# AwesomePeiweiPan/Droid-SLAM_Reserch

Hardware: AMD Instinct MI355X
Metric: BA update iters/sec (2000-edge equivalents; 256 keyframes, 48x64) (higher is better)
Workload: dtype f32; 1 GPU; 256-keyframe / 2000-edge global BA, 48x64, t0=1, lm=1e-5 ep=1e-2 (BASELINE configs[2]); edges_total=2000, solve=fp64 dense Cholesky on device, chol_failed=False

## Files before the change

droid-slam_reserch_amd/csrc/ba_internal.hpp:

```cpp
#pragma once
#include <hip/hip_runtime.h>
#include <stddef.h>
#include <stdint.h>

namespace droid {

constexpr int LIN_THREADS = 256;
constexpr int LIN_PPT = 2;
constexpr int LIN_CP = LIN_THREADS * LIN_PPT;
constexpr int LIN_WAVES = LIN_THREADS / 64;
constexpr int CHOL_NB = 64;
__host__ __device__ inline int chol_ld(int n) { return (n + 1 + 15) & ~15; }
__host__ __device__ inline size_t chol_flag_words(int n) { return 2 * ((size_t)(n + 1 + CHOL_NB - 1) / CHOL_NB) + 8; }
__host__ __device__ inline int chol_tile_index(int nrb, int bi, int bj) { return bj * nrb - bj * (bj - 1) / 2 + (bi - bj); }
__host__ __device__ inline size_t chol_tiles(int n) {
  const int nb = (n + CHOL_NB - 1) / CHOL_NB, nrb = (n + 1 + CHOL_NB - 1) / CHOL_NB;
  return (size_t)chol_tile_index(nrb, nb, nb);
}
__host__ __device__ inline size_t chol_mbuf_offset(int n) { return ((size_t)(n + CHOL_NB - 1) / CHOL_NB) * CHOL_NB * CHOL_NB; }
__host__ __device__ inline size_t chol_lfin_offset(int n) { return 2 * chol_mbuf_offset(n); }
__host__ __device__ inline size_t chol_ldiag_doubles(int n) { return chol_lfin_offset(n) + chol_tiles(n) * CHOL_NB * CHOL_NB; }

__host__ __device__ inline size_t pk_colbase(int n, int J) {
  return (size_t)CHOL_NB * ((size_t)J * (size_t)(n + 1) - (size_t)CHOL_NB * (size_t)J * (size_t)(J - 1) / 2);
}
__host__ __device__ inline int pk_width(int n, int J) { return (n - CHOL_NB * J) < CHOL_NB ? (n - CHOL_NB * J) : CHOL_NB; }
__host__ __device__ inline size_t pk_total(int n) {
  if (n <= 0) return 0;
  const int nb = (n + CHOL_NB - 1) / CHOL_NB;
  return pk_colbase(n, nb - 1) + (size_t)(n + 1 - CHOL_NB * (nb - 1)) * (size_t)pk_width(n, nb - 1);
}
__host__ __device__ inline size_t pk_index(int n, int gi, int gj) {
  const int J = gj / CHOL_NB;
  return pk_colbase(n, J) + (size_t)(gi - CHOL_NB * J) * (size_t)pk_width(n, J) + (size_t)(gj - CHOL_NB * J);
}
__host__ __device__ inline unsigned pk_index32(int n, int gi, int gj) {
  const int J = gj >> 6, c0 = J << 6;
  const int w = (n - c0) < CHOL_NB ? (n - c0) : CHOL_NB;
  return (unsigned)(CHOL_NB * (J * (n + 1) - (CHOL_NB / 2) * J * (J - 1)) + (gi - c0) * w + (gj - c0));
}

enum { HDR_STATUS = 0, HDR_M = 1, HDR_CHOL_FAIL = 2, HDR_NENT = 3, HDR_NWORK = 4,
       HDR_NC1 = 5, HDR_NC2 = 6,
       HDR_WORDS = 16 };
enum { STATUS_BAD_INDEX = 1, STATUS_ETA_ROWS = 2, STATUS_CHOL_FAIL = 4, STATUS_CHOL_STALL = 8 };

struct BaView {
  int E, nbuf, H, W, HW;
  int t0, t1, P, M;
  int n, ld;
  int nch;
  int own0, own1;
  int motion_only;
  int* hdr;
  int* slot_of;
  int* kx;
  int* seg_ptr;
  int* seg_edge;
  int* cursor;
  int* ent_ptr;
  int* ent_row;
  int* ent_pose;
  int* wk_ptr;
  int* order;
  int* xtmp;
  int* cls_list;
  int* gt_ptr;
  double* Gpart;
  int s2_split;
  float* Hpart;
  float* Q;
  float* w;
  float* Erows;
  float* Ebuf;
  float* sy_part[2];
  int sy_ns[2];
  int wide;
  int zsplit;
  float* zpart;
  double* sys;
  double* psys;
  int packed;
  double* xsol;
  float* dx;
  int* bs_flags;
  double* ldiag;
  int* hint;
  int hint_tag;
  int* ov_ready;
  float* pose_snap;
};

constexpr int SY_WGS = 1024;
constexpr int S2_WGS = 1536;
constexpr int SF_WGS = 1536;
constexpr int LIN_WGS = 1536;
constexpr int LIN_ZERO_WGS = 192;
constexpr int SF_TP = 64;
constexpr int SW_MID = 256;
constexpr int SW_BIG = 512;
constexpr int tri_tiles16(int rows) { return (rows / 16) * (rows / 16 + 1) / 2; }
constexpr int SY_T1 = tri_tiles16(SW_MID), SY_T2 = tri_tiles16(SW_BIG);
constexpr int SY_FOLD_GROUPS = SY_T1 / 4;

inline size_t ba_carve(BaView& v, void* ws, int E, int nbuf, int H, int W, int t0, int t1, int M) {
  v.E = E; v.nbuf = nbuf; v.H = H; v.W = W; v.HW = H * W;
  v.t0 = t0; v.t1 = t1; v.P = t1 - t0; v.M = M;
  v.n = 6 * v.P; v.ld = chol_ld(v.n);
  v.nch = (v.HW + LIN_CP - 1) / LIN_CP;
  v.own0 = 0; v.own1 = nbuf; v.motion_only = 0;
  v.hint = nullptr; v.hint_tag = 0;
  size_t off = 0;
  char* base = static_cast<char*>(ws);
  auto take = [&](size_t bytes) {
    void* p = base ? base + off : nullptr;
    off += (bytes + 255) & ~size_t(255);
    return p;
  };
  v.hdr = static_cast<int*>(take(sizeof(int) * HDR_WORDS));
  v.slot_of = static_cast<int*>(take(sizeof(int) * (nbuf + 1)));
  v.kx = static_cast<int*>(take(sizeof(int) * (nbuf + 1)));
  v.seg_ptr = static_cast<int*>(take(sizeof(int) * (nbuf + 2)));
  v.seg_edge = static_cast<int*>(take(sizeof(int) * (E + 1)));
  v.cursor = static_cast<int*>(take(sizeof(int) * (nbuf + 2)));
  v.ent_ptr = static_cast<int*>(take(sizeof(int) * (nbuf + 2)));
  v.ent_row = static_cast<int*>(take(sizeof(int) * ((size_t)M + E + 1)));
  v.ent_pose = static_cast<int*>(take(sizeof(int) * ((size_t)M + E + 1)));
  v.wk_ptr = static_cast<int*>(take(sizeof(int) * (nbuf + 2)));
  v.order = static_cast<int*>(take(sizeof(int) * (nbuf + 2)));
  v.gt_ptr = static_cast<int*>(take(sizeof(int) * (nbuf + 2)));
  v.cls_list = static_cast<int*>(take(sizeof(int) * 2 * (nbuf + 2)));
  v.xtmp = static_cast<int*>(take(sizeof(int) * 3 * ((size_t)E + 1)));
  v.Hpart = static_cast<float*>(take(sizeof(float) * ((size_t)E * v.nch * LIN_WAVES * 32 + 32)));
  v.Q = static_cast<float*>(take(sizeof(float) * ((size_t)M * v.HW + 4)));
  v.w = static_cast<float*>(take(sizeof(float) * ((size_t)M * v.HW + 4)));
  v.Erows = nullptr;
  v.wide = (M > 0 && (long)E >= 12l * M && (v.HW % 32) == 0) ? 1 : 0;
  v.Ebuf = nullptr;
  if (v.wide) v.Ebuf = static_cast<float*>(take(sizeof(float) * (6 * ((size_t)M + E) * v.HW + 64)));
  v.sy_part[0] = v.sy_part[1] = nullptr;
  v.sy_ns[0] = v.sy_ns[1] = 0;
  if (v.wide) {
    const int stages = v.HW / 32;
    int nsw = (SY_WGS + M - 1) / M, nsb = (256 + 4 * M - 1) / (4 * M);
    nsw = nsw < 2 ? 2 : (nsw > stages ? stages : nsw);
    nsb = nsb < 2 ? 2 : (nsb > stages ? stages : nsb);
    if (nsw > 16) nsw = 16;
    if (nsb > 16) nsb = 16;
    v.sy_ns[0] = nsw; v.sy_ns[1] = nsb;
    v.sy_part[0] = static_cast<float*>(take(sizeof(float) * ((size_t)M * nsw * SY_T1 * 256 + 64)));
    v.sy_part[1] = static_cast<float*>(take(sizeof(float) * ((size_t)M * nsb * SY_T2 * 256 + 64)));
  }
  v.zsplit = 1;
  if (M > 0) {
    const int z = LIN_WGS / (M * v.nch);
    v.zsplit = z < 1 ? 1 : (z > 8 ? 8 : z);
  }
  v.zpart = nullptr;
  if (v.zsplit > 1) v.zpart = static_cast<float*>(take(sizeof(float) * ((size_t)v.zsplit * M * 8 * v.HW + 64)));
  v.s2_split = 1;
  v.Gpart = nullptr;
  if (M > 0) {
    const int ptiles = (v.HW + 63) / 64;
    int ns = S2_WGS / M;
    v.s2_split = ns < 1 ? 1 : (ns > ptiles ? ptiles : ns);
    size_t tiles = (size_t)E * 7 / 4 + (size_t)M + 1;
    if (tiles > (size_t)28 * M) tiles = (size_t)28 * M;
    v.Gpart = static_cast<double*>(take(sizeof(double) * (tiles * v.s2_split * 256 + 64)));
  }
  v.sys = static_cast<double*>(take(sizeof(double) * ((size_t)(v.n + 1) * v.ld + 8)));
  v.psys = static_cast<double*>(take(sizeof(double) * (pk_total(v.n) + 8)));
  v.packed = 0;
  v.xsol = static_cast<double*>(take(sizeof(double) * ((size_t)v.ld + 1)));
  v.bs_flags = static_cast<int*>(take(sizeof(int) * chol_flag_words(v.n)));
  v.ldiag = static_cast<double*>(take(sizeof(double) * chol_ldiag_doubles(v.n)));
  v.dx = static_cast<float*>(take(sizeof(float) * ((size_t)v.n + 8)));
  v.ov_ready = static_cast<int*>(take(sizeof(int) * ((size_t)(v.n + 1 + CHOL_NB - 1) / CHOL_NB + 8)));
  v.pose_snap = static_cast<float*>(take(sizeof(float) * 7 * (size_t)nbuf));
  return off;
}

__host__ __device__ inline int solver_preset_words(const BaView& v) {
  return (int)((reinterpret_cast<const char*>(v.bs_flags) - reinterpret_cast<const char*>(v.xsol)) / 4 +
               (long)chol_flag_words(v.n));
}
__host__ __device__ inline int solver_preset_tiles(const BaView& v) { return v.n > 0 ? (int)chol_tiles(v.n) : 0; }

struct BaLaunchPlan {
  int zero_wgs;
  int asm_units;
  dim3 schur2;
  int sf_split;
  dim3 syrk[2], fold;
};
inline BaLaunchPlan ba_launch_plan(const BaView& v) {
  BaLaunchPlan p;
  p.zero_wgs = LIN_ZERO_WGS;
  p.asm_units = v.E > 0 ? v.E + (solver_preset_words(v) + 1023) / 1024 + solver_preset_tiles(v) : 0;
  p.schur2 = dim3(v.M + (p.asm_units + 4 * v.s2_split - 1) / (4 * v.s2_split), v.s2_split);
  const int tiles = (v.HW + SF_TP - 1) / SF_TP, ns = SF_WGS / (v.M > 0 ? v.M : 1);
  p.sf_split = ns < 1 ? 1 : (ns > tiles ? tiles : ns);
  p.syrk[0] = dim3(v.M, v.sy_ns[0], 1);
  p.syrk[1] = dim3(v.M, v.sy_ns[1], 4);
  p.fold = dim3(v.M, SY_FOLD_GROUPS, 2);
  return p;
}

struct CholSystem {
  double* S; int n, ld; double* x; int* flags; double* ldiag; int* fail;
  explicit CholSystem(const BaView& v)
      : S(v.sys), n(v.n), ld(v.ld), x(v.xsol), flags(v.bs_flags), ldiag(v.ldiag), fail(v.hdr + HDR_CHOL_FAIL) {}
  CholSystem(double* scratch, int n, double* x, int* fail);
  static size_t scratch_doubles(int n);
};

void launch_wave_reduce32_test(const float* in, float* out, hipStream_t s);
void launch_lin_test(const BaView& v, const float* poses, const float* disps, const float* intr, const float* sens,
                     const float* targets, const float* weights, const float* eta, const int64_t* ii, const int64_t* jj,
                     bool motion_only, bool ragged, hipStream_t s);
void launch_prep(const BaView& v, const int64_t* ii, const int64_t* jj, hipStream_t s);
void launch_unpack_system(const BaView& v, hipStream_t s);
void launch_build_stage(const BaView& v, const BaLaunchPlan& plan, const float* poses, const float* disps,
                        const float* intr, const float* sens, const float* targets, const float* weights,
                        const float* eta, const int64_t* ii, const int64_t* jj, bool motion_only,
                        int stage, hipStream_t s);
void launch_update(const BaView& v, float* poses, float* disps, const float* intr, const float* weights,
                   const int64_t* ii, const int64_t* jj, const double* x, float* dx_out, float* dz_out,
                   bool motion_only, hipStream_t s, int* status_mirror = nullptr);
void launch_chol_preset(const CholSystem& c, hipStream_t s);
bool launch_chol_factor(const CholSystem& c, double lm, double ep, hipStream_t s);
void launch_chol_backsolve(const CholSystem& c, bool factor_single, hipStream_t s);
void launch_chol_solve(const CholSystem& c, double lm, double ep, hipStream_t s, bool preset_done);

void launch_unpack_cols(const BaView& v, int J0, int J1, double lm, double ep, int epoch, hipStream_t s);
bool launch_chol_factor_overlap(const CholSystem& c, const int* ready, int epoch, hipStream_t s);
bool chol_overlap_available(int n);

}
```

droid-slam_reserch_amd/csrc/chol.hip:

```cpp
#include <hip/hip_runtime.h>
#include <mutex>

#include <cstdint>
#include <cstdlib>

#include "ba_internal.hpp"
#include "launchers.hpp"

namespace droid {

constexpr int NB = CHOL_NB;

#ifdef CHOL_STAMPS
__device__ unsigned long long g_chol_stamps[64 * 16];
__device__ unsigned long long g_bs_stamps[64 * 8];
__shared__ unsigned long long g_chol_lstamps[16];
extern "C" int droid_debug_chol_stamps(unsigned long long* out) {
  return (int)hipMemcpyFromSymbol(out, HIP_SYMBOL(g_chol_stamps), sizeof(unsigned long long) * 64 * 16);
}
extern "C" int droid_debug_bs_stamps(unsigned long long* out) {
  return (int)hipMemcpyFromSymbol(out, HIP_SYMBOL(g_bs_stamps), sizeof(unsigned long long) * 64 * 8);
}
#define STEP_STAMP(slot)                                                                                      \
  do { if (threadIdx.x == 0 && panel && (blockIdx.x < 2))                                                      \
// ... 821 lines not shown
  int *done = flags, *dver = flags + nrb, *abortf = flags + 2 * nrb;
  const int G = (int)gridDim.x, wg = (int)blockIdx.x, t = (int)threadIdx.x;
  const int total = (int)chol_tiles(n);
  {
    int cs = 0;
    for (int j = 0; j < nb; j++) {
      if (j >= 1 && (cs % G) == wg) cfp_publish_diag(dver, j, 0);
      cs += nrb - j;
    }
  }
  OV_STAMP_ENTERED();
  if (t == 0) {
    int nt = 0, cj = 0, cs = 0;
    for (int idx = wg; idx < total && nt < MAXT; idx += G) {
      while (idx >= cs + (nrb - cj)) {
        cs += nrb - cj;
        cj++;
      }
      s_ti[nt] = cj + (idx - cs);
      s_tj[nt] = cj;
      s_nx[nt] = cfp_first_step(cj);
      nt++;
    }
    s_nt = nt;
  }
  __syncthreads();
  while (true) {
    if (t < 64) {
      int pick = -1, spins = 0, klast = -2;
      bool ok = true;
      const int nt = s_nt;
      while (true) {
        bool any_left = false;
        for (int i = 0; i < nt; i++) {
          const int bi = s_ti[i], bj = s_tj[i], k = s_nx[i];
          if (k > bj - 1) continue;
          any_left = true;
          const bool panel = (bj == k + 1);
          const CfpInput in = cfp_input<true>(t, bi, bj, k, panel, done, dver, ready, epoch, Ldiag, n);
          const int fv = (in.flag == nullptr) ? 0x7fffffff : cfp_load(in.flag);
          const bool sat = (in.slot != nullptr) ? __double_as_longlong(gload<true>(in.slot)) != CFP_TAG : fv >= in.need;
          if (__all(sat)) {
            pick = i;
            klast = k;
            if (cfp_waits_for_done(bj, k, panel)) {
              const int d0 = __shfl(fv, 0), d1 = (bj != bi) ? __shfl(fv, 1) : d0;
              const int cok = (min(d0, d1) - 3) >> 2;
              klast = max(k, min(cok, bj - 3));
            }
            break;
          }
        }
        if (!any_left) pick = -2;
        if (pick != -1) break;
        if (++spins > (CFP_SPIN_LIMIT << 2) || ((spins & 63) == 0 && __any(cfp_load(abortf) == 1))) {
          ok = false;
          break;
        }
        __builtin_amdgcn_s_sleep(4);
      }
      if (t == 0) {
        s_pick = ok ? pick : -3;
        s_klast = klast;
        if (!ok) cfp_report_stall(fail, abortf);
      }
    }
    __syncthreads();
    const int pick = s_pick;
    if (pick < 0) return;
    const int bi = __builtin_amdgcn_readfirstlane(s_ti[pick]), bj = __builtin_amdgcn_readfirstlane(s_tj[pick]);
    const int k = __builtin_amdgcn_readfirstlane(s_nx[pick]);
    const int klast = __builtin_amdgcn_readfirstlane(s_klast);
    chol_tile_persist<true>(S, n, ld, k, bi, bj, fail, lm, ep, Ldiag, done, abortf, k == cfp_first_step(bj), klast);
    OV_STAMP_DIAG(bi, bj, k);
    if (bj != k + 1 && bi == bj) cfp_publish_diag(dver, bj, max(k, klast) + 1);
    __syncthreads();
    if (t == 0) s_nx[pick] = max(k, klast) + 1;
    __syncthreads();
  }
}

__global__ __launch_bounds__(256) void chol_backsolve_kernel(double* __restrict__ S, int n, int ld,
                                                             int k, double* __restrict__ x) {
  __shared__ double L[NB * LDP];
  __shared__ double xk[NB];
  const int t = threadIdx.x;
  const int c0 = k * NB;
  const int wk = min(NB, n - c0);
  load_tile64(DROID_LDS(L), (const gbl_f64*)S, ld, c0, c0, c0, c0 + wk, c0 + wk, true, 1.0);
  __syncthreads();
  if (t < 64) {
    double z = (t < wk) ? S[(size_t)n * ld + c0 + t] : 0.0;
    const double rinv = 1.0 / L[t * LDP + t];
#pragma unroll
    for (int i = NB - 1; i >= 0; i--) {
      const double xi = readlane_f64(z * rinv, i);
      z = (t == i) ? xi : ((t < i) ? fma(-L[i * LDP + t], xi, z) : z);
    }
    xk[t] = z;
  }
  __syncthreads();
  if (blockIdx.x == 0) {
    if (t < wk) x[c0 + t] = xk[t];
    return;
  }
  const int c = (blockIdx.x - 1) * 256 + t;
  if (c < c0) {
    double s4[4] = {0.0, 0.0, 0.0, 0.0};
    const double* col = S + (size_t)c0 * ld + c;
#pragma unroll
    for (int r = 0; r < NB; r += 16) {
      double v[16];
#pragma unroll
      for (int u = 0; u < 16; u++) v[u] = (r + u < wk) ? col[(size_t)(r + u) * ld] : 0.0;
#pragma unroll
      for (int u = 0; u < 16; u++) s4[u & 3] = fma(v[u], xk[r + u], s4[u & 3]);
    }
    S[(size_t)n * ld + c] -= (s4[0] + s4[1]) + (s4[2] + s4[3]);
  }
}

constexpr int BSP_MAX_BLOCKS = 200;
constexpr long long BSP_SENTINEL = -1LL;

__device__ __forceinline__ void load_tile64_w123(lds_f64* __restrict__ dst, const gbl_f64* __restrict__ S,
                                                 int ld, int r0, int c0, int row_end, int col_end) {
  const int t = threadIdx.x - 64;
  f64x2 v[11];
#pragma unroll
  for (int it = 0; it < 11; it++) {
    const int idx2 = it * 192 + t;
    const int i = idx2 >> 5, j = (idx2 & 31) * 2;
    const bool ok = (idx2 < 2048) && (r0 + i < row_end) && (c0 + j < col_end);
    const gbl_f64* p = S + (size_t)(ok ? r0 + i : 0) * ld + (ok ? c0 + j : 0);
    v[it] = *(const gbl_f64x2*)p;
    if (!ok) v[it] = (f64x2){0.0, 0.0};
    else if (c0 + j + 1 >= col_end) v[it][1] = 0.0;
  }
#pragma unroll
  for (int it = 0; it < 11; it++) {
    const int idx2 = it * 192 + t;
    if (idx2 < 2048) {
      const int i = idx2 >> 5, j = (idx2 & 31) * 2;
      *(lds_f64x2*)(&dst[i * LDP + j]) = v[it];
    }
  }
}

template <bool FAST>
__global__ __launch_bounds__(256) void chol_backsolve_persistent_kernel(
    double* __restrict__ S, int n, int ld, double* __restrict__ x, int* __restrict__ err,
    const double* __restrict__ Ldiag) {
  __shared__ double Ld[NB * LDP];
  __shared__ double Tt[2][NB * LDP];
  __shared__ double xk[NB];
  __shared__ int dead;
  const int t = threadIdx.x;
  const int nb = gridDim.x;
  const int j = blockIdx.x;
  const int c0 = j * NB;
  const int wj = min(NB, n - c0);
  BS_STAMP(0);
  if (t == 0) dead = 0;
  if (FAST) load_tile64(DROID_LDS(Ld), (const gbl_f64*)Ldiag + (size_t)j * NB * NB, NB, 0, 0, 0, wj, wj, true, 1.0);
  else load_tile64(DROID_LDS(Ld), (const gbl_f64*)S, ld, c0, c0, c0, c0 + wj, c0 + wj, true, 1.0);
  double z = (t < wj) ? S[(size_t)n * ld + c0 + t] : 0.0;
  int cur = 0;
  auto load_k = [&](double* dst, int k) {
    if (FAST && k == j + 1)
      load_tile64_w123(DROID_LDS(dst), (const gbl_f64*)Ldiag + chol_mbuf_offset(n) + (size_t)j * NB * NB, NB, 0, 0, NB, NB);
    else
      load_tile64_w123(DROID_LDS(dst), (const gbl_f64*)S, ld, k * NB, c0, n, c0 + wj);
  };
  if (j < nb - 1 && t >= 64) load_k(Tt[0], nb - 1);
  __syncthreads();
  double Lcol[NB];
  double Wcol[16];
  if (t < 64) {
#pragma unroll
    for (int i = FAST ? 16 : 0; i < NB; i++) Lcol[i] = Ld[i * LDP + t];
    if (FAST) {
      const int pb = t >> 4, br = pb == 3 ? 1 : 0, bc = pb == 3 ? 2 : pb + 1;
      const double* Wg = Ldiag + (size_t)j * NB * NB + (size_t)(16 * br) * NB + 16 * bc + (t & 15);
#pragma unroll
      for (int c = 0; c < 16; c++) Wcol[c] = Wg[c * NB];
    }
  }
  auto poll_matvec = [&](int k, const double (&Tc)[NB]) -> double {
    const int gi = k * NB + t;
    double xv = 0.0;
    if (gi < n) {
      int spins = 0;
      while (true) {
        xv = __hip_atomic_load(&x[gi], __ATOMIC_RELAXED, __HIP_MEMORY_SCOPE_AGENT);
        if (__double_as_longlong(xv) != BSP_SENTINEL) break;
        if (++spins > (1 << 22)) {
          dead = 1;
          atomicMax(err, 2);
          xv = 0.0;
          break;
        }
        __builtin_amdgcn_s_sleep(1);
      }
    }
    if (k == j + 1) BS_STAMP(1);
    xk[t] = xv;
    double a0 = 0.0, a1 = 0.0, a2 = 0.0, a3 = 0.0;
#pragma unroll
    for (int r = 0; r < NB; r += 4) {
      const f64x2 x01 = *(const lds_f64x2*)&DROID_LDS(xk)[r], x23 = *(const lds_f64x2*)&DROID_LDS(xk)[r + 2];
      a0 = fma(Tc[r + 0], x01[0], a0);
      a1 = fma(Tc[r + 1], x01[1], a1);
      a2 = fma(Tc[r + 2], x23[0], a2);
      a3 = fma(Tc[r + 3], x23[1], a3);
    }
    return (a0 + a1) + (a2 + a3);
  };
  const int klast = FAST ? j + 2 : j + 1;
  for (int k = nb - 1; k >= klast; k--) {
    if (t >= 64) {
      if (k - 1 > j) load_k(Tt[cur ^ 1], k - 1);
    } else {
      double Tc[NB];
      {
        const double* T = Tt[cur];
#pragma unroll
        for (int r = 0; r < NB; r++) Tc[r] = T[r * LDP + t];
      }
      z -= poll_matvec(k, Tc);
    }
    cur ^= 1;
    if (!FAST && k == j + 1) {
      BS_STAMP(2);
      break;
    }
    __syncthreads();
    if (dead) return;
  }
  BS_STAMP(3);
  if (t < 64) {
    double xsol = 0.0;
    double Mc[NB];
    if (FAST && j < nb - 1) {
      const double* T = Tt[cur];
#pragma unroll
      for (int r = 0; r < NB; r++) Mc[r] = T[r * LDP + t];
    }
    const double rinv = FAST ? 0.0 : 1.0 / Ld[t * LDP + t];
    const int rr = t & 15, rowb = t >> 4;
#define DROID_BS_STEP(B, II)                                                                            \
    {                                                                                                  \
      double zr = z * rinv, xi;                                                                        \
      asm volatile("s_nop 1\n\tv_mov_b64_dpp %0, %1 row_newbcast:" #II " row_mask:0xf bank_mask:0xf"   \
                   : "=v"(xi) : "v"(zr));                                                              \
      z = fma(-Lcol[16 * B + II], xi, z);   \
      xsol = (rr == II) ? xi : xsol;                                                                   \
    }
#define DROID_BS_WTERM(ACC, C)                                                                          \
    asm volatile("v_fmac_f64_dpp %0, %1, %2 row_newbcast:" #C " row_mask:0xf bank_mask:0xf"             \
                 : "+v"(ACC) : "v"(z), "v"(Wcol[C]));
#define DROID_BS_BLOCK(B)                                                                               \
    if (rowb == B) {                                                                                   \
      if (FAST) {                                                                                      \
        double xw = 0.0, xv2 = 0.0;                                                                    \
        asm volatile("s_nop 1" : "+v"(z));                                                             \
        DROID_BS_WTERM(xw, 0) DROID_BS_WTERM(xv2, 1) DROID_BS_WTERM(xw, 2) DROID_BS_WTERM(xv2, 3)      \
        DROID_BS_WTERM(xw, 4) DROID_BS_WTERM(xv2, 5) DROID_BS_WTERM(xw, 6) DROID_BS_WTERM(xv2, 7)      \
        DROID_BS_WTERM(xw, 8) DROID_BS_WTERM(xv2, 9) DROID_BS_WTERM(xw, 10) DROID_BS_WTERM(xv2, 11)    \
        DROID_BS_WTERM(xw, 12) DROID_BS_WTERM(xv2, 13) DROID_BS_WTERM(xw, 14) DROID_BS_WTERM(xv2, 15)  \
        xsol = xw + xv2;                                                                               \
      } else {                                                                                         \
        DROID_BS_STEP(B, 15) DROID_BS_STEP(B, 14) DROID_BS_STEP(B, 13) DROID_BS_STEP(B, 12)            \
        DROID_BS_STEP(B, 11) DROID_BS_STEP(B, 10) DROID_BS_STEP(B, 9) DROID_BS_STEP(B, 8)              \
        DROID_BS_STEP(B, 7) DROID_BS_STEP(B, 6) DROID_BS_STEP(B, 5) DROID_BS_STEP(B, 4)                \
        DROID_BS_STEP(B, 3) DROID_BS_STEP(B, 2) DROID_BS_STEP(B, 1) DROID_BS_STEP(B, 0)                \
      }                                                                                                \
      xk[t] = xsol;                                                                                    \
    }                                                                                                  \
    if (B > 0 && rowb < B) {                                                                           \
      double u0 = 0.0, u1 = 0.0;                                                                       \
      _Pragma("unroll") for (int ii = 0; ii < 16; ii += 2) {                                           \
        const f64x2 xx = *(const lds_f64x2*)&DROID_LDS(xk)[16 * B + ii];                                \
        u0 = fma(Lcol[16 * B + ii], xx[0], u0);                                                        \
        u1 = fma(Lcol[16 * B + ii + 1], xx[1], u1);                                                    \
      }                                                                                                \
      z -= u0 + u1;                                                                                    \
    }
    DROID_BS_BLOCK(3)
    DROID_BS_BLOCK(2)
    DROID_BS_BLOCK(1)
    DROID_BS_BLOCK(0)
#undef DROID_BS_BLOCK
#undef DROID_BS_WTERM
#undef DROID_BS_STEP
    BS_STAMP(2);
    if (FAST && j < nb - 1) xsol -= poll_matvec(j + 1, Mc);
    if (__double_as_longlong(xsol) == BSP_SENTINEL) xsol = __longlong_as_double(0x7ff8000000000000LL);
    BS_STAMP(4);
    if (t < wj) __hip_atomic_store(&x[c0 + t], xsol, __ATOMIC_RELAXED, __HIP_MEMORY_SCOPE_AGENT);
    BS_STAMP(5);
  }
}

struct CholSwitches {
  bool multi_launch;
  bool cooperative;
  bool force_bs_refusal;
  int grid;
  int overlap_reserve;
};
static const CholSwitches& chol_switches() {
  const auto is_set = [](const char* name) { return getenv(name) != nullptr; };
  const auto number = [](const char* name, int unset) { const char* v = getenv(name); return v ? atoi(v) : unset; };
  static const CholSwitches sw = {is_set("DROID_CHOL_MULTI_LAUNCH"), number("DROID_CHOL_COOPERATIVE", 0) != 0,
                                  is_set("DROID_CHOL_FORCE_BS_REFUSAL"), number("DROID_CHOL_GRID", 0),
                                  number("DROID_OVERLAP_RESERVE_CUS", 32)};
  return sw;
}

struct PersistState {
  hipStream_t last = nullptr;
  hipEvent_t ev = nullptr;
  bool any = false;
  int resident = -1;
};
static PersistState g_persist[64];
static std::mutex g_persist_mu;

static int chol_resident_workgroups() {
  int dev = 0;
  if (hipGetDevice(&dev) != hipSuccess || dev < 0 || dev >= 64) return 0;
  std::lock_guard<std::mutex> lock(g_persist_mu);
  int& cached = g_persist[dev].resident;
  if (cached < 0) {
    int occ = 0;
    hipDeviceProp_t prop;
    const bool known = hipGetDeviceProperties(&prop, dev) == hipSuccess &&
        hipOccupancyMaxActiveBlocksPerMultiprocessor(&occ, chol_factor_persistent_kernel<false>, 512, 0) == hipSuccess;
    cached = known ? occ * prop.multiProcessorCount : 0;
  }
  return cached;
}

static int chol_single_launch(const CholSystem& c) {
  const int nb = (c.n + NB - 1) / NB;
  if (chol_switches().multi_launch || nb < 2 || (c.ld % 16) != 0 || (reinterpret_cast<uintptr_t>(c.S) % 128) != 0) return 0;
  const int resident = chol_resident_workgroups();
  return (resident >= 8 && chol_tiles(c.n) <= (size_t)10 * resident) ? resident : 0;
}

static bool launch_spinning_grid(const void* fn, int workgroups, int threads, void** args, hipStream_t s, bool refuse = false) {
  std::lock_guard<std::mutex> lock(g_persist_mu);
  int dev = 0;
  if (hipGetDevice(&dev) == hipSuccess && dev >= 0 && dev < 64) {
    PersistState& st = g_persist[dev];
    if (st.any && st.last != s) {
      if (!st.ev && hipEventCreateWithFlags(&st.ev, hipEventDisableTiming) != hipSuccess) st.ev = nullptr;
      if (st.ev && hipEventRecord(st.ev, st.last) == hipSuccess) (void)hipStreamWaitEvent(s, st.ev, 0);
      (void)hipGetLastError();
    }
    st.last = s, st.any = true;
  }
  if (!chol_switches().cooperative) {
    (void)hipLaunchKernel(fn, dim3(workgroups), dim3(threads), args, 0, s);
    return true;
  }
  if (!refuse && hipLaunchCooperativeKernel(fn, dim3(workgroups), dim3(threads), args, 0, s) == hipSuccess) return true;
  (void)hipGetLastError();
  return false;
}

__global__ __launch_bounds__(256) void chol_ldiag_to_sys_kernel(double* __restrict__ S, int n, int ld,
                                                                const double* __restrict__ Ldiag) {
  const int j = blockIdx.x, c0 = j * NB, wk = min(NB, n - c0);
  for (int idx = threadIdx.x; idx < NB * NB; idx += blockDim.x) {
    const int i = idx / NB, c = idx % NB;
    if (i < wk && c <= i) S[(size_t)(c0 + i) * ld + c0 + c] = Ldiag[(size_t)j * NB * NB + idx];
  }
}

static bool launch_factor_grid(const void* fn, CholSystem c, double lm, double ep, const int* ready, int epoch, int cap,
                               hipStream_t s) {
  void* args[] = {&c.S, &c.n, &c.ld, &c.fail, &lm, &ep, &c.flags, &c.ldiag, &ready, &epoch};
  return launch_spinning_grid(fn, chol_tiles(c.n) < (size_t)cap ? (int)chol_tiles(c.n) : cap, 512, args, s);
}

static int chol_overlap_cap(int n) {
  const CholSwitches& sw = chol_switches();
  const int nb = (n + NB - 1) / NB;
  if (n <= 0 || sw.cooperative || sw.multi_launch || nb < 2) return 0;
  const int resident = chol_resident_workgroups();
  if (resident < 8 || chol_tiles(n) > (size_t)10 * resident) return 0;
  const int cap = resident - (sw.overlap_reserve > 0 ? sw.overlap_reserve : 0);
  return (cap >= 8 && chol_tiles(n) <= (size_t)10 * cap) ? cap : 0;
}
bool chol_overlap_available(int n) { return chol_overlap_cap(n) > 0; }

bool launch_chol_factor_overlap(const CholSystem& c, const int* ready, int epoch, hipStream_t s) {
  if (!ready || (c.ld % 16) != 0 || (reinterpret_cast<uintptr_t>(c.S) % 128) != 0) return false;
  const int cap = chol_overlap_cap(c.n);
  if (cap == 0) return false;
  return launch_factor_grid((const void*)chol_factor_persistent_kernel<true>, c, 0.0, 0.0, ready, epoch, cap, s);
}

bool launch_chol_factor(const CholSystem& c, double lm, double ep, hipStream_t s) {
  if (c.n <= 0) return false;
  if (int cap = chol_single_launch(c)) {
    const int grid = chol_switches().grid;
    if (grid >= 8 && grid < cap) cap = grid;
    if (launch_factor_grid((const void*)chol_factor_persistent_kernel<false>, c, lm, ep, nullptr, 0, cap, s)) return true;
  }
  const int nb = (c.n + NB - 1) / NB;
  const int nrb = (c.n + 1 + NB - 1) / NB;
  for (int k = -1; k + 1 < nb; k++)
    hipLaunchKernelGGL(chol_step_kernel, dim3(nrb - k - 1, k < 0 ? 2 : nb - k - 1), dim3(512), 0, s, c.S, c.n,
                       c.ld, k, c.fail, lm, ep);
  return false;
}

void launch_chol_backsolve(const CholSystem& c, bool factor_single, hipStream_t s) {
  const int nb = (c.n + NB - 1) / NB;
  if (nb >= 2 && nb <= BSP_MAX_BLOCKS) {
    CholSystem a = c;
    const double* ld_arg = factor_single ? c.ldiag : nullptr;
    void* args[] = {&a.S, &a.n, &a.ld, &a.x, &a.fail, &ld_arg};
    const void* fn = factor_single ? (const void*)chol_backsolve_persistent_kernel<true>
                                   : (const void*)chol_backsolve_persistent_kernel<false>;
    if (launch_spinning_grid(fn, nb, 256, args, s, chol_switches().force_bs_refusal)) return;
  }
  if (factor_single)
    hipLaunchKernelGGL(chol_ldiag_to_sys_kernel, dim3(nb), dim3(256), 0, s, c.S, c.n, c.ld, c.ldiag);
  for (int k = nb - 1; k >= 0; k--) {
    const int c0 = k * NB;
    hipLaunchKernelGGL(chol_backsolve_kernel, dim3(1 + (c0 + 255) / 256), dim3(256), 0, s, c.S, c.n,
                       c.ld, k, c.x);
  }
}

void launch_chol_preset(const CholSystem& c, hipStream_t s) {
  (void)hipMemsetAsync(c.fail, 0, sizeof(int), s);
  const size_t xbytes = sizeof(double) * (size_t)c.n, fbytes = sizeof(int) * chol_flag_words(c.n);
  const char* xb = reinterpret_cast<const char*>(c.x);
  const char* fb = reinterpret_cast<const char*>(c.flags);
  if (fb >= xb + xbytes && fb - xb <= (ptrdiff_t)(xbytes + 4096)) {
    (void)hipMemsetAsync(c.x, 0xFF, (size_t)(fb - xb) + fbytes, s);
  } else {
    (void)hipMemsetAsync(c.x, 0xFF, xbytes, s);
    (void)hipMemsetAsync(c.flags, 0xFF, fbytes, s);
  }
  (void)hipMemsetAsync(c.ldiag + chol_lfin_offset(c.n), 0xFF, sizeof(double) * chol_tiles(c.n) * NB * NB, s);
}

void launch_chol_solve(const CholSystem& c, double lm, double ep, hipStream_t s, bool preset_done) {
  if (c.n <= 0) return;
  if (!preset_done) launch_chol_preset(c, s);
  const bool single = launch_chol_factor(c, lm, ep, s);
  launch_chol_backsolve(c, single, s);
}

size_t CholSystem::scratch_doubles(int n) {
  if (n <= 0) return 0;
  return (size_t)(n + 1) * chol_ld(n) + chol_ldiag_doubles(n) + (chol_flag_words(n) + 1) / 2 + 16;
}
CholSystem::CholSystem(double* scratch, int n_, double* x_, int* fail_)
    : S(scratch), n(n_), ld(chol_ld(n_)), x(x_), fail(fail_) {
  ldiag = S + (size_t)(n + 1) * ld;
  flags = reinterpret_cast<int*>(ldiag + chol_ldiag_doubles(n));
}

__global__ void chol_pack_kernel(const double* __restrict__ A, const double* __restrict__ b,
                                 double* __restrict__ S, int n, int ld) {
  const size_t idx = (size_t)blockIdx.x * blockDim.x + threadIdx.x;
  if (idx >= (size_t)(n + 1) * ld) return;
  const int r = (int)(idx / ld), c = (int)(idx % ld);
  double val = 0.0;
  if (r < n && c < n) val = A[(size_t)r * n + c];
  else if (r == n && c < n) val = b[c];
  S[idx] = val;
}

void launch_chol_pack(const double* A, const double* b, double* S, int n, int ld, hipStream_t s) {
  const size_t tot = (size_t)(n + 1) * ld;
  hipLaunchKernelGGL(chol_pack_kernel, dim3((unsigned)((tot + 255) / 256)), dim3(256), 0, s, A, b,
                     S, n, ld);
}

}
```

Before: 2048 iters/s.

## Add paired-column persistent backsolve kernel with 512 threads per workgroup

Adds a new backward-substitution kernel in which each 512-thread workgroup owns two adjacent 64-column blocks instead of one. This halves the number of spinning workgroups and the cross-workgroup dependency chain. The near off-diagonal tiles are preloaded and multiplied by precomputed diagonal inverses with f64 MFMA, so the coupling between the two columns is resolved locally. It is enabled by default whenever the single-launch factor path is used. In exchange it uses more registers and LDS per workgroup, and the polling and sentinel logic is more complex.

```diff
diff --git a/droid-slam_reserch_amd/csrc/ba_internal.hpp b/droid-slam_reserch_amd/csrc/ba_internal.hpp
--- a/droid-slam_reserch_amd/csrc/ba_internal.hpp
+++ b/droid-slam_reserch_amd/csrc/ba_internal.hpp
@@ -20,6 +20,9 @@
 __host__ __device__ inline size_t chol_mbuf_offset(int n) { return ((size_t)(n + CHOL_NB - 1) / CHOL_NB) * CHOL_NB * CHOL_NB; }
 __host__ __device__ inline size_t chol_lfin_offset(int n) { return 2 * chol_mbuf_offset(n); }
 __host__ __device__ inline size_t chol_ldiag_doubles(int n) { return chol_lfin_offset(n) + chol_tiles(n) * CHOL_NB * CHOL_NB; }
+__host__ __device__ inline int chol_bs_pairs_grid(int nb) { return (nb + 1) / 2; }
+__host__ __device__ inline int chol_bs_pairs_owner(int col) { return col / 2; }
+__host__ __device__ inline int chol_bs_pairs_first(int wg) { return 2 * wg; }
 
 __host__ __device__ inline size_t pk_colbase(int n, int J) {
   return (size_t)CHOL_NB * ((size_t)J * (size_t)(n + 1) - (size_t)CHOL_NB * (size_t)J * (size_t)(J - 1) / 2);
diff --git a/droid-slam_reserch_amd/csrc/chol.hip b/droid-slam_reserch_amd/csrc/chol.hip
--- a/droid-slam_reserch_amd/csrc/chol.hip
+++ b/droid-slam_reserch_amd/csrc/chol.hip
@@ -1147,19 +1147,304 @@
   }
 }
 
+#ifdef CHOL_STAMPS
+#define BS_STAMP_W(slot, wv) do { if (threadIdx.x == 64 * (wv) && blockIdx.x < 64) g_bs_stamps[blockIdx.x * 8 + (slot)] = wall_clock64(); } while (0)
+#else
+#define BS_STAMP_W(slot, wv) do { } while (0)
+#endif
+
+struct BspTileRegs { f64x2 v[4]; };
+__device__ __forceinline__ BspTileRegs bsp_tile_issue(const gbl_f64* __restrict__ src, size_t pitch, int rows_valid) {
+  const int t = threadIdx.x;
+  BspTileRegs r;
+#pragma unroll
+  for (int it = 0; it < 4; it++) {
+    const int idx2 = it * 512 + t, i = idx2 >> 5, j = (idx2 & 31) * 2;
+    const bool ok = i < rows_valid;
+    r.v[it] = *(const gbl_f64x2*)(src + (ok ? (size_t)i * pitch + j : 0));
+    if (!ok) r.v[it] = (f64x2){0.0, 0.0};
+  }
+  return r;
+}
+__device__ __forceinline__ void bsp_tile_store(lds_f64* __restrict__ dst, const BspTileRegs& r) {
+  const int t = threadIdx.x;
+#pragma unroll
+  for (int it = 0; it < 4; it++) {
+    const int idx2 = it * 512 + t, i = idx2 >> 5, j = (idx2 & 31) * 2;
+    *(lds_f64x2*)(&dst[i * LDP + j]) = r.v[it];
+  }
+}
+
+constexpr int BSP_DC = 10 * 256;
+__device__ __forceinline__ int bsp_dc_source(int e) {
+  const int blk = e >> 7, i = (e & 127) >> 3, j = (e & 7) * 2;
+  int br, bc;
+  if (blk < 6) {
+    br = blk < 1 ? 1 : (blk < 3 ? 2 : 3);
+    bc = blk - br * (br - 1) / 2;
+  } else {
+    br = blk == 9 ? 1 : 0;
+    bc = blk == 9 ? 2 : blk - 5;
+  }
+  return (16 * br + i) * NB + 16 * bc + j;
+}
+
+__device__ __forceinline__ void bsp_times_inverse(lds_f64* T, const lds_f64* D, int g, int lane) {
+  const int fr = lane & 15, fg = lane >> 4;
+#pragma unroll
+  for (int q = 3; q >= 0; q--) {
+    lds_f64* Cq = &T[(16 * g) * LDP + 16 * q];
+    f64x4 acc;
+#pragma unroll
+    for (int i = 0; i < 4; i++) acc[i] = Cq[(fg + 4 * i) * LDP + fr];
+#pragma unroll
+    for (int s2 = q + 1; s2 < 4; s2++)
+#pragma unroll
+      for (int kk = 0; kk < 16; kk += 4)
+        acc = __builtin_amdgcn_mfma_f64_16x16x4f64(-T[(16 * g + fr) * LDP + 16 * s2 + kk + fg],
+                                                   D[(s2 * (s2 - 1) / 2 + q) * 256 + (kk + fg) * 16 + fr], acc, 0, 0, 0);
+#pragma unroll
+    for (int i = 0; i < 4; i++) Cq[(fg + 4 * i) * LDP + fr] = acc[i];
+    f64x4 m = {0.0, 0.0, 0.0, 0.0};
+#pragma unroll
+    for (int kk = 0; kk < 16; kk += 4)
+      m = __builtin_amdgcn_mfma_f64_16x16x4f64(Cq[fr * LDP + kk + fg], D[(6 + q) * 256 + (kk + fg) * 16 + fr], m, 0, 0, 0);
+#pragma unroll
+    for (int i = 0; i < 4; i++) Cq[(fg + 4 * i) * LDP + fr] = m[i];
+  }
+}
+
+template <int NN>
+__device__ __forceinline__ double bsp_dot(const double* col, const lds_f64* xs) {
+  double a0 = 0.0, a1 = 0.0, a2 = 0.0, a3 = 0.0;
+#pragma unroll
+  for (int r = 0; r < NN; r += 4) {
+    const f64x2 x01 = *(const lds_f64x2*)&xs[r], x23 = *(const lds_f64x2*)&xs[r + 2];
+    a0 = fma(col[r + 0], x01[0], a0);
+    a1 = fma(col[r + 1], x01[1], a1);
+    a2 = fma(col[r + 2], x23[0], a2);
+    a3 = fma(col[r + 3], x23[1], a3);
+  }
+  return (a0 + a1) + (a2 + a3);
+}
+
+__global__ __launch_bounds__(512) void chol_backsolve_pairs_kernel(
+    double* __restrict__ S_, int n, int ld, double* __restrict__ x, int* __restrict__ err,
+    const double* __restrict__ Ldiag_) {
+  __shared__ double Dc[2][BSP_DC];
+  __shared__ double Nt[3][NB * LDP];
+  __shared__ double xs[8][NB];
+  __shared__ double far_part[8][NB];
+  __shared__ double near_part[8][NB];
+  __shared__ double us[2][NB];
+  __shared__ int dead;
+  const gbl_f64* const S = (const gbl_f64*)S_;
+  const gbl_f64* const Ldiag = (const gbl_f64*)Ldiag_;
+  const int t = threadIdx.x, w = t >> 6, l = t & 63;
+  const int nb = (n + NB - 1) / NB, G = gridDim.x, J = blockIdx.x;
+  const int b = chol_bs_pairs_first(J), a = b + 1;
+  const bool has_a = a < nb;
+  const bool above = a + 1 < nb;
+  const bool above2 = a + 2 < nb;
+  const int ch = w & 1, rq = w >> 1;
+  lds_f64* const xw = DROID_LDS(xs[w]);
+  BS_STAMP_W(0, 0);
+  if (t == 0) dead = 0;
+
+  const int ra = (a + 1) * NB, rb = (a + 2) * NB;
+  BspTileRegs t0, t1, t2;
+  f64x2 dreg[5];
+  if (above) {
+    t1 = bsp_tile_issue(S + (size_t)ra * ld + (size_t)b * NB, ld, n - ra);
+    if (above2) {
+      t2 = bsp_tile_issue(S + (size_t)rb * ld + (size_t)b * NB, ld, n - rb);
+      t0 = bsp_tile_issue(S + (size_t)rb * ld + (size_t)a * NB, ld, n - rb);
+    }
+#pragma unroll
+    for (int it = 0; it < 5; it++) {
+      const int idx2 = it * 512 + t, which = idx2 >= BSP_DC / 2 ? 1 : 0;
+      dreg[it] = *(const gbl_f64x2*)(Ldiag + (size_t)(b + which) * NB * NB + bsp_dc_source(idx2 - which * (BSP_DC / 2)));
+    }
+  }
+
+  double keep[NB];
+  {
+    const gbl_f64* base = Ldiag;
+    int row_lo = 0, col_lo = l, row_hi = 0, used = 0;
+    if (w == 4 || (w == 5 && has_a)) {
+      const int pb = l >> 4;
+      base = Ldiag + (size_t)(b + w - 4) * NB * NB;
+      row_lo = pb == 3 ? 16 : 0;
+      col_lo = 16 * (pb == 3 ? 2 : pb + 1) + (l & 15);
+      used = NB;
+    } else if (w == 6 && has_a) {
+      base = Ldiag + chol_mbuf_offset(n) + (size_t)b * NB * NB;
+      used = NB;
+    } else if (ch == 1 && rq < 2 && above) {
+      base = Ldiag + chol_mbuf_offset(n) + (size_t)a * NB * NB;
+      row_lo = row_hi = 32 * rq;
+      used = 32;
+    }
+#pragma unroll
+    for (int i = 0; i < NB; i++) {
+      keep[i] = 0.0;
+      if (i < used) keep[i] = base[(size_t)((i < 16 ? row_lo : row_hi) + i) * NB + (i < 16 ? col_lo : l)];
+    }
+  }
+  double z = 0.0;
+  if ((w == 4 || (w == 5 && has_a)) && (b + w - 4) * NB + l < n) z = S[(size_t)n * ld + (b + w - 4) * NB + l];
+
+  if (above) {
+    bsp_tile_store(DROID_LDS(Nt[1]), t1);
+    if (above2) {
+      bsp_tile_store(DROID_LDS(Nt[2]), t2);
+      bsp_tile_store(DROID_LDS(Nt[0]), t0);
+    }
+#pragma unroll
+    for (int it = 0; it < 5; it++) *(lds_f64x2*)&DROID_LDS(Dc[0])[2 * (it * 512 + t)] = dreg[it];
+    __syncthreads();
+    if (w < 4) {
+      bsp_times_inverse(DROID_LDS(Nt[1]), DROID_LDS(Dc[0]), w, l);
+      if (above2) bsp_times_inverse(DROID_LDS(Nt[0]), DROID_LDS(Dc[1]), w, l);
+    } else if (above2) {
+      bsp_times_inverse(DROID_LDS(Nt[2]), DROID_LDS(Dc[0]), w - 4, l);
+    }
+  }
+  BS_STAMP_W(1, 0);
+
+  auto poll = [&](int gi, int lanes) -> double {
+    double xv = 0.0;
+    if (l < lanes && gi + l < n) {
+      int spins = 0;
+      while (true) {
+        xv = __hip_atomic_load(&x[gi + l], __ATOMIC_RELAXED, __HIP_MEMORY_SCOPE_AGENT);
+        if (__double_as_longlong(xv) != BSP_SENTINEL) break;
+        if (++spins > (1 << 22)) {
+          *(volatile int*)&dead = 1;
+          atomicMax(err, 2);
+          xv = 0.0;
+          break;
+        }
+        __builtin_amdgcn_s_sleep(1);
+      }
+    }
+    return xv;
+  };
+
+  double far = 0.0;
+  for (int P = G - 1; P >= J + 2; P--) {
+    if (*(volatile int*)&dead) break;
+    const int r0 = 2 * P * NB + 32 * rq;
+    const gbl_f64* col = S + (size_t)(b + ch) * NB + l;
+    double Tc[32];
+#pragma unroll
+    for (int r = 0; r < 32; r++) {
+      const int row = r0 + r;
+      Tc[r] = col[(size_t)(row < n ? row : n - 1) * ld];
+      if (row >= n) Tc[r] = 0.0;
+    }
+    const double xv = poll(r0, 32);
+    if (l < 32) xw[l] = xv;
+    far += bsp_dot<32>(Tc, xw);
+  }
+  DROID_LDS(far_part[w])[l] = far;
+  BS_STAMP_W(2, 0);
+  __syncthreads();
+  if (dead) return;
+
+  if (w == 4 || (w == 5 && has_a)) {
+    const int c = w - 4;
+    z -= (far_part[c][l] + far_part[2 + c][l]) + (far_part[4 + c][l] + far_part[6 + c][l]);
+    const int rowb = l >> 4;
+    double xsol = 0.0;
+#define DROID_BSP_WTERM(ACC, C)                                                                         \
+    asm volatile("v_fmac_f64_dpp %0, %1, %2 row_newbcast:" #C " row_mask:0xf bank_mask:0xf"             \
+                 : "+v"(ACC) : "v"(z), "v"(keep[C]));
+#define DROID_BSP_BLOCK(B)                                                                              \
+    if (rowb == B) {                                                                                   \
+      double xw0 = 0.0, xw1 = 0.0;                                                                     \
+      asm volatile("s_nop 1" : "+v"(z));                                                               \
+      DROID_BSP_WTERM(xw0, 0) DROID_BSP_WTERM(xw1, 1) DROID_BSP_WTERM(xw0, 2) DROID_BSP_WTERM(xw1, 3)  \
+      DROID_BSP_WTERM(xw0, 4) DROID_BSP_WTERM(xw1, 5) DROID_BSP_WTERM(xw0, 6) DROID_BSP_WTERM(xw1, 7)  \
+      DROID_BSP_WTERM(xw0, 8) DROID_BSP_WTERM(xw1, 9) DROID_BSP_WTERM(xw0, 10) DROID_BSP_WTERM(xw1, 11) \
+      DROID_BSP_WTERM(xw0, 12) DROID_BSP_WTERM(xw1, 13) DROID_BSP_WTERM(xw0, 14) DROID_BSP_WTERM(xw1, 15) \
+      xsol = xw0 + xw1;                                                                                \
+      xw[l] = xsol;                                                                                    \
+    }                                                                                                  \
+    if (B > 0 && rowb < B) {                                                                           \
+      double u0 = 0.0, u1 = 0.0;                                                                       \
+      _Pragma("unroll") for (int ii = 0; ii < 16; ii += 2) {                                           \
+        const f64x2 xx = *(const lds_f64x2*)&xw[16 * B + ii];                                           \
+        u0 = fma(keep[16 * B + ii], xx[0], u0);                                                        \
+        u1 = fma(keep[16 * B + ii + 1], xx[1], u1);                                                    \
+      }                                                                                                \
+      z -= u0 + u1;                                                                                    \
+    }
+    DROID_BSP_BLOCK(3)
+    DROID_BSP_BLOCK(2)
+    DROID_BSP_BLOCK(1)
+    DROID_BSP_BLOCK(0)
+#undef DROID_BSP_BLOCK
+#undef DROID_BSP_WTERM
+    DROID_LDS(us[c])[l] = xsol;
+    BS_STAMP_W(3, 4);
+  }
+
+  double near = 0.0;
+  if (above && (rq < 2 || above2)) {
+    double Nc[32];
+    if (ch == 1 && rq < 2) {
+#pragma unroll
+      for (int r = 0; r < 32; r++) Nc[r] = keep[r];
+    } else {
+      const lds_f64* T = DROID_LDS(ch == 1 ? Nt[0] : (rq < 2 ? Nt[1] : Nt[2])) + (32 * (rq & 1)) * LDP + l;
+#pragma unroll
+      for (int r = 0; r < 32; r++) Nc[r] = T[r * LDP];
+    }
+    const double xv = poll((a + 1) * NB + 32 * rq, 32);
+    BS_STAMP_W(4, 0);
+    if (l < 32) xw[l] = xv;
+    near = bsp_dot<32>(Nc, xw);
+  }
+  DROID_LDS(near_part[w])[l] = near;
+  __syncthreads();
+  if (dead) return;
+  BS_STAMP_W(5, 6);
+  if (w == 6 || (w == 7 && has_a)) {
+    const auto publish = [&](int c0, double v) {
+      if (__double_as_longlong(v) == BSP_SENTINEL) v = __longlong_as_double(0x7ff8000000000000LL);
+      if (c0 + l < n) __hip_atomic_store(&x[c0 + l], v, __ATOMIC_RELAXED, __HIP_MEMORY_SCOPE_AGENT);
+    };
+    double xb = us[0][l] - ((near_part[0][l] + near_part[2][l]) + (near_part[4][l] + near_part[6][l]));
+    if (has_a) {
+      const double xa = us[1][l] - ((near_part[1][l] + near_part[3][l]) + (near_part[5][l] + near_part[7][l]));
+      if (w == 7) {
+        publish(a * NB, xa);
+        return;
+      }
+      xw[l] = (a * NB + l < n) ? xa : 0.0;
+      xb -= bsp_dot<NB>(keep, xw);
+    }
+    BS_STAMP_W(6, 6);
+    publish(b * NB, xb);
+    BS_STAMP_W(7, 6);
+  }
+}
+
 struct CholSwitches {
   bool multi_launch;
   bool cooperative;
   bool force_bs_refusal;
   int grid;
   int overlap_reserve;
+  bool bs_pairs;
 };
 static const CholSwitches& chol_switches() {
   const auto is_set = [](const char* name) { return getenv(name) != nullptr; };
   const auto number = [](const char* name, int unset) { const char* v = getenv(name); return v ? atoi(v) : unset; };
   static const CholSwitches sw = {is_set("DROID_CHOL_MULTI_LAUNCH"), number("DROID_CHOL_COOPERATIVE", 0) != 0,
                                   is_set("DROID_CHOL_FORCE_BS_REFUSAL"), number("DROID_CHOL_GRID", 0),
-                                  number("DROID_OVERLAP_RESERVE_CUS", 32)};
+                                  number("DROID_OVERLAP_RESERVE_CUS", 32), number("DROID_CHOL_BS_PAIRS", 1) != 0};
   return sw;
 }
 
@@ -1263,15 +1548,23 @@
   return false;
 }
 
+extern "C" int droid_debug_bs_pairs_map(int nb, int* owner) {
+  for (int j = 0; j < nb; j++) owner[j] = chol_bs_pairs_owner(j);
+  return chol_bs_pairs_grid(nb);
+}
+
 void launch_chol_backsolve(const CholSystem& c, bool factor_single, hipStream_t s) {
   const int nb = (c.n + NB - 1) / NB;
   if (nb >= 2 && nb <= BSP_MAX_BLOCKS) {
     CholSystem a = c;
     const double* ld_arg = factor_single ? c.ldiag : nullptr;
     void* args[] = {&a.S, &a.n, &a.ld, &a.x, &a.fail, &ld_arg};
-    const void* fn = factor_single ? (const void*)chol_backsolve_persistent_kernel<true>
+    const bool pairs = factor_single && chol_switches().bs_pairs;
+    const void* fn = pairs ? (const void*)chol_backsolve_pairs_kernel
+                   : factor_single ? (const void*)chol_backsolve_persistent_kernel<true>
                                    : (const void*)chol_backsolve_persistent_kernel<false>;
-    if (launch_spinning_grid(fn, nb, 256, args, s, chol_switches().force_bs_refusal)) return;
+    if (launch_spinning_grid(fn, pairs ? chol_bs_pairs_grid(nb) : nb, pairs ? 512 : 256, args, s,
+                             chol_switches().force_bs_refusal)) return;
   }
   if (factor_single)
     hipLaunchKernelGGL(chol_ldiag_to_sys_kernel, dim3(nb), dim3(256), 0, s, c.S, c.n, c.ld, c.ldiag);
```

New measurement: 2090 iters/s (median of 6 runs). 1.02x the previous value.
